# Liam-Eagen/BulletproofsPP

Measured on AMD Instinct MI355X. Metric: msm_scalar_point_pairs_per_sec, higher is better.
Workload: dtype u256 modular integer (Fq: 10x26-bit lazy limbs, Fr: 8x32-bit limbs); 1 GPU; pedersen_msm_2^20_secp256k1; pairs_per_gpu=1048576, window_bits=auto, algorithm=signed-digit Pippenger, affine in / XYZZ buckets

## Files before the change

bulletproofspp_amd/capi.py:

```python
from __future__ import annotations

import ctypes as C
import os
from typing import Optional, Sequence, Tuple

import numpy as np

_HERE = os.path.dirname(os.path.abspath(__file__))
NUM_STAGES = 6
STAGE_NAMES = ["digits", "sort", "acc_points", "acc_records", "reduce", "finish"]

SYMBOLS = [
    "bppp_ctx_create", "bppp_ctx_destroy", "bppp_ctx_set_stream", "bppp_last_error", "bppp_version",
    "bppp_msm", "bppp_msm_device", "bppp_msm_batch_device", "bppp_sum_points", "bppp_rational_reduce",
    "bppp_fold_points", "bppp_fold_points_device", "bppp_rational_reduce_eis", "bppp_fold_points_eis_device",
    "bppp_norm_round_sums_device", "bppp_lin_round_sums_device",
    "bppp_norm_round_openings_device", "bppp_lin_round_openings_device",
    "bppp_fold_scalars_device", "bppp_tensor_device", "bppp_batch_inverse_device",
    "bppp_nl_create", "bppp_nl_destroy", "bppp_nl_lengths", "bppp_nl_round_commit", "bppp_nl_round_collapse",
    "bppp_nl_get_witness", "bppp_nl_download", "bppp_nl_verify", "bppp_nl_verify_batch_device", "bppp_nl_prove", "bppp_nl_verify_challenges",
    "bppp_nlb_create", "bppp_nlb_destroy", "bppp_nlb_lengths", "bppp_nlb_round_commit", "bppp_nlb_round_collapse", "bppp_nlb_get_witness",
    "bppp_ip_create", "bppp_ip_destroy", "bppp_ip_lengths", "bppp_ip_round_commit", "bppp_ip_round_collapse", "bppp_ip_get_witness", "bppp_ip_verify", "bppp_ip_verify_batch_device",
    "bppp_lift_x_device", "bppp_device_alloc", "bppp_device_free", "bppp_upload", "bppp_download", "bppp_host_alloc", "bppp_host_free",
    "bppp_profile_enable", "bppp_profile_read",
# ... 214 lines not shown
    lib = C.CDLL(p)
    vp, sz, i = C.c_void_p, C.c_size_t, C.c_int
    lib.bppp_test_fe_op.argtypes = [vp, i, i, vp, vp, sz, vp]
    lib.bppp_test_point_op.argtypes = [vp, i, vp, vp, sz, vp]
    lib.bppp_test_point_quad.argtypes = [vp, i, vp, vp, sz, vp, vp]
    lib.bppp_test_fq_pair.argtypes = [vp, i, vp, vp, vp, vp, sz, vp]
    lib.bppp_test_point_chain.argtypes = [vp, i, vp, vp, sz, vp, vp]
    lib.bppp_test_mulmod_rate.argtypes = [vp, i, C.POINTER(C.c_double)]
    lib.bppp_test_last_mixed_msm_terms.argtypes = [vp, C.POINTER(C.c_uint64)]
    lib.bppp_test_last_sort_ranges.argtypes = [vp, C.POINTER(C.c_int)]
    lib.bppp_test_last_scatter_one_read.argtypes = [vp, C.POINTER(C.c_int)]
    lib.bppp_test_last_acc_sized.argtypes = [vp, C.POINTER(C.c_int)]
    lib.bppp_test_last_acc_fq29.argtypes = [vp, C.POINTER(C.c_int)]
    lib.bppp_test_fq29_op.argtypes = [vp, i, vp, vp, sz, vp, vp]
    lib.bppp_test_madd29_chain.argtypes = [vp, vp, vp, sz, sz, vp, vp]
    lib.bppp_test_last_windows.argtypes = [vp, C.POINTER(C.c_int)]
    lib.bppp_test_rp_last_verify_counts.argtypes = [vp, C.POINTER(C.c_uint64), C.POINTER(C.c_uint64)]
    lib.bppp_test_rp_last_block_counts.argtypes = [vp] + [C.POINTER(C.c_uint64)] * 4
    lib.bppp_test_rp_set_each_chunk.argtypes = [vp, sz]
    lib.bppp_test_rp_set_tally_short_max.argtypes = [vp, sz]
    lib.bppp_test_rp_set_tally_piece.argtypes = [vp, sz]
    lib.bppp_test_rp_set_tally_chunk.argtypes = [vp, sz]
    lib.bppp_test_rp_set_flat_chunk.argtypes = [vp, sz]
    lib.bppp_test_rp_excess_mul.argtypes = [vp, sz, vp, vp, vp]
    lib.bppp_test_rp_excess_mul2.argtypes = [vp, sz, vp, vp, vp, vp, vp]
    lib.bppp_test_rp_witness_device.argtypes = [vp, sz, vp, vp, vp, vp, vp, vp, vp, vp, vp]
    lib.bppp_test_points_from_seed_chunked.argtypes = [vp, C.c_char_p, sz, C.c_uint64, sz, sz, vp, C.POINTER(C.c_uint64)]
    lib.bppp_test_seed_lift_digests.argtypes = [vp, C.c_char_p, sz, vp, vp, vp]
    lib.bppp_test_rp_decode_device.argtypes = [vp, sz, C.c_char_p, C.c_char_p, vp, vp, vp, vp, vp, vp]
    lib.bppp_test_comb_create.argtypes = [vp, vp, sz, i, C.POINTER(vp)]
# ... 411 lines not shown
```

bulletproofspp_amd/csrc/capi.hip:

```cpp
#include <stdlib.h>
#include <string.h>
#include "ctx.hpp"
#include "hostmath.hpp"
#include "hosteis.hpp"

namespace bppp {
int msm_run(bppp_ctx *, const void *, const void *, size_t, size_t, int, int, uint64_t *);
int fold_points_run(bppp_ctx *, const uint64_t *, int, const uint64_t *, int, const void *, size_t, void *);
int norm_round_sums_run(bppp_ctx *, const void *, size_t, const uint64_t *, uint64_t *, uint64_t *);
int lin_round_sums_run(bppp_ctx *, const void *, const void *, size_t, uint64_t *, uint64_t *);
int round_openings_run(bppp_ctx *, const void *, size_t, int, const uint64_t *, const uint64_t *, void *, void *);
int fold_scalars_run(bppp_ctx *, const uint64_t *, const uint64_t *, const void *, size_t, void *);
int tensor_run(bppp_ctx *, const uint64_t *, size_t, const uint64_t *, const uint64_t *, size_t, void *);
int lift_x_run(bppp_ctx *, const void *, size_t, void *);
int batch_inverse_run(bppp_ctx *, const void *, size_t, int, void *);
int fold_points_eis_run(bppp_ctx *, const uint64_t *, const int *, const uint64_t *, const int *, const void *, size_t, void *);

void ctx_retain(bppp_ctx *ctx) { ctx->refs.fetch_add(1); }
void ctx_release(bppp_ctx *ctx) {
  if (ctx->refs.fetch_sub(1) != 1) return;
  hipSetDevice(ctx->device);
  hipStreamSynchronize(ctx->stream);
  if (ctx->aux_stream) hipStreamSynchronize(ctx->aux_stream);
  if (ctx->ws) hipFree(ctx->ws);
// ... 20 lines not shown
  lacc = env_int("BPPP_LACC", 0);
  window_batched = env_int("BPPP_WINDOW_BATCHED", 0);
  comb_wpe = env_int("BPPP_COMB_WPE", 0);
  comb_rows_waves = env_int("BPPP_COMB_ROWS_WAVES", 0);
  if (const char *e = getenv("BPPP_COMB_ROWS_MIN_MB")) comb_rows_min_bytes = (size_t)strtoull(e, nullptr, 10) << 20;
  small_c = env_int("BPPP_MSM_SMALL_C", 0);
  small_len = env_int("BPPP_MSM_SMALL_LEN", 0);
  small_max = env_int("BPPP_MSM_SMALL_MAX", 0);
  hist_ch = env_int("BPPP_HIST_CH", 0);
  no_small = env_flag("BPPP_MSM_NO_SMALL");
  no_balance = env_flag("BPPP_MSM_NO_BALANCE");
  sort_ranges = env_int("BPPP_SORT_RANGES", sort_ranges);
  scatter_one_read = env_switch("BPPP_SCATTER_ONE_READ", scatter_one_read);
  acc_sized = env_switch("BPPP_ACC_SIZED", acc_sized);
  acc_fq29 = env_switch("BPPP_ACC_FQ29", acc_fq29);
}
namespace bppp {
int ctx_aux(bppp_ctx *ctx) {
  if (ctx->aux_stream) return BPPP_OK;
  BPPP_HIP(ctx, hipStreamCreateWithFlags(&ctx->aux_stream, hipStreamNonBlocking));
  BPPP_HIP(ctx, hipEventCreateWithFlags(&ctx->aux_fork, hipEventDisableTiming));
  BPPP_HIP(ctx, hipEventCreateWithFlags(&ctx->aux_join, hipEventDisableTiming));
  return BPPP_OK;
}
void ctx_drain(bppp_ctx *ctx) {
  if (ctx_closed(ctx)) return;
  hipStreamSynchronize(ctx->stream);
  if (ctx->aux_stream) hipStreamSynchronize(ctx->aux_stream);
  (void)hipGetLastError();
}
// ... 289 lines not shown
```

bulletproofspp_amd/csrc/ctx.hpp:

```cpp
#pragma once
#include <hip/hip_runtime.h>
#include <stdint.h>
#include <atomic>
#include <string>
#include <vector>
#include "../../include/bppp.h"
#include "msm_plan.hpp"

struct CombLast {
  int route = -1;
  int heavy_first = 0;
  uint32_t parts = 0, tparts = 0, wsplit = 0;
  uint32_t chunks = 0, clen = 0, join_lanes = 0;
};

struct bppp_ctx {
  MsmTune tune;
  std::atomic<int> refs{1};
  std::atomic<bool> closed{false};
  int device = 0;
  hipStream_t stream = nullptr;
  hipStream_t own_stream = nullptr;
  hipStream_t aux_stream = nullptr;
  hipEvent_t aux_fork = nullptr, aux_join = nullptr;
// ... 6 lines not shown
  void *pre_acc_arg = nullptr;
  void *pinned = nullptr;
  size_t pinned_bytes = 0;
  bool profile = false;
  double stage_ms[BPPP_NUM_STAGES] = {0, 0, 0, 0, 0, 0};
  uint64_t calls = 0;
  hipEvent_t ev[BPPP_NUM_STAGES + 1] = {};
  bool ev_ready = false;
  void *mix = nullptr;
  size_t mix_bytes = 0;
  uint64_t last_mixed_terms = 0;
  int last_sort_ranges = -1;
  int last_scatter_one_read = -1;
  int last_acc_sized = -1;
  int last_acc_fq29 = -1;
  int last_windows = -1;
  CombLast last_comb;
  size_t sort_lds_set = 0;
};

namespace bppp {

inline int fail(bppp_ctx *ctx, int code, const std::string &msg) {
  if (ctx) ctx->err = msg;
  return code;
}
#define BPPP_HIP(ctx, call)                                                                    \
  do {                                                                                         \
    hipError_t _e = (call);                                                                    \
    if (_e != hipSuccess)                                                                      \
// ... 16 lines not shown
```

bulletproofspp_amd/csrc/ec29.hip.h:

```cpp
#pragma once
#include "ec.hip.h"
#include "fq29.hip.h"

namespace bppp {

struct aff29 { fq29 x, y; };
struct xyzz29 { fq29 X, Y, ZZ, ZZZ; };

BPPP_DI bool aff29_is_inf(const aff29 &p) { return fq29_all_zero(p.x) && fq29_all_zero(p.y); }
BPPP_DI bool xyzz29_is_inf(const xyzz29 &p) { return fq29_all_zero(p.ZZ); }
BPPP_DI xyzz29 xyzz29_inf() { xyzz29 r; r.X = fq29_zero(); r.Y = fq29_zero(); r.ZZ = fq29_zero(); r.ZZZ = fq29_zero(); return r; }
BPPP_DI xyzz29 xyzz29_from_aff(const aff29 &p) {
  xyzz29 r; r.X = p.x; r.Y = p.y;
  r.ZZ = fq29_zero(); r.ZZ.n[0] = aff29_is_inf(p) ? 0u : 1u; r.ZZZ = r.ZZ;
  return r;
}
BPPP_DI aff29 aff29_cneg(const aff29 &p, bool neg) {
  aff29 r; r.x = p.x;
  const fq29 ny = fq29_neg<1>(p.y);
  const bool inf = aff29_is_inf(p);
#pragma unroll
  for (int i = 0; i < 9; i++) r.y.n[i] = (neg && !inf) ? ny.n[i] : p.y.n[i];
  return r;
}
// ... 18 lines not shown
  if (fq29_weak_is_zero(Pd)) {
    if (fq29_weak_is_zero(R)) acc = xyzz29_dbl_aff(q); else acc = xyzz29_inf();
    return;
  }
  const fq29 PP = fq29_sqr(Pd), PPP = fq29_mul(Pd, PP), Q = fq29_mul(acc.X, PP);
  const fq29 X3 = fq29_sub<3>(fq29_sqr(R), fq29_add(PPP, fq29_mul_int(Q, 2)));
  const fq29 Y3 = fq29_sub<1>(fq29_mul(R, fq29_sub<5>(Q, X3)), fq29_mul(acc.Y, PPP));
  acc.ZZ = fq29_mul(acc.ZZ, PP); acc.ZZZ = fq29_mul(acc.ZZZ, PPP);
  acc.X = X3; acc.Y = Y3;
}

BPPP_DI xyzz xyzz29_to_xyzz(const xyzz29 &a) {
  xyzz r; r.X = fq29_to_fq26(a.X); r.Y = fq29_to_fq26(a.Y); r.ZZ = fq29_to_fq26(a.ZZ); r.ZZZ = fq29_to_fq26(a.ZZZ);
  return r;
}

}
```

bulletproofspp_amd/csrc/fq26.hip.h:

```cpp
#pragma once
#include "fe.hip.h"
#include "modinv.hip.h"

namespace bppp {

struct fq { uint32_t n[10]; };

static constexpr uint32_t FQ_M26 = 0x3FFFFFFu, FQ_M22 = 0x3FFFFFu;
static constexpr uint32_t FQ_R0 = 0x3D10u, FQ_R1 = 0x400u;

BPPP_DI uint32_t fq_plimb(int i) { return i == 0 ? 0x3FFFC2Fu : i == 1 ? 0x3FFFFBFu : i == 9 ? FQ_M22 : FQ_M26; }

BPPP_DI fq fq_zero() { fq r; for (int i = 0; i < 10; i++) r.n[i] = 0; return r; }
BPPP_DI fq fq_one() { fq r = fq_zero(); r.n[0] = 1; return r; }
BPPP_DI bool fq_all_zero(const fq &a) {
  uint32_t o = 0;
#pragma unroll
  for (int i = 0; i < 10; i++) o |= a.n[i];
  return o == 0;
}

BPPP_DI uint64_t fq_madc(uint32_t x, uint32_t y, uint64_t acc) { uint64_t r = (uint64_t)x * y + acc; asm("" : "+v"(r)); return r; }
BPPP_DI uint32_t fq_sreg(uint32_t v) { asm("" : "+s"(v)); return v; }
BPPP_DI void fq_mul_tail(fq &r, uint64_t c, uint32_t t9, uint64_t u9, uint32_t u8) {
  c += (uint64_t)t9 + u9 * FQ_R0 + (uint64_t)u8 * FQ_R1;
  r.n[9] = (uint32_t)c & FQ_M22;
  const uint64_t top = (c >> 22) + ((u9 * FQ_R1) << 4);
  c = (uint64_t)r.n[0] + top * 0x3D1u; r.n[0] = (uint32_t)c & FQ_M26; c >>= 26;
  c += (uint64_t)r.n[1] + (top << 6); r.n[1] = (uint32_t)c & FQ_M26; c >>= 26;
  c += r.n[2]; r.n[2] = (uint32_t)c & FQ_M26; c >>= 26;
  r.n[3] += (uint32_t)c;
}
BPPP_DI fq fq_mul(const fq &a, const fq &b) {
  const uint32_t R0 = fq_sreg(FQ_R0), R1 = fq_sreg(FQ_R1);
  uint64_t d = 0;
#pragma unroll
  for (int i = 0; i <= 9; i++) d = fq_madc(a.n[i], b.n[9 - i], d);
  const uint32_t t9 = (uint32_t)d & FQ_M26; d >>= 26;
// ... 47 lines not shown
    if (k) c = fq_madc(u[k - 1], R1, c);
    r.n[k] = (uint32_t)c & FQ_M26; c >>= 26;
  }
  fq_mul_tail(r, c, t9, u9, u[8]);
  return r;
}

template <bool SQ> BPPP_DI constexpr int fq_col_n(int k) {
  return SQ ? ((k + 1) / 2 - (k > 9 ? k - 9 : 0)) + ((k & 1) == 0 ? 1 : 0) : (k < 9 ? k : 9) - (k > 9 ? k - 9 : 0) + 1;
}
template <bool SQ> BPPP_DI uint64_t fq_col_step(const fq &a, const fq &b, int k, int j, uint64_t acc) {
  const int i = (k > 9 ? k - 9 : 0) + j;
  if (SQ) return 2 * i < k ? fq_madc(b.n[i], a.n[k - i], acc) : fq_madc(a.n[k / 2], a.n[k / 2], acc);
  return fq_madc(a.n[i], b.n[k - i], acc);
}
BPPP_DI void fq_fence() { __builtin_amdgcn_sched_barrier(0); }
template <bool SQ1, bool SQ2> BPPP_DI void fq_pair(const fq a, const fq b_, const fq c, const fq d_, fq &r1, fq &r2) {
  const uint32_t R0 = fq_sreg(FQ_R0), R1 = fq_sreg(FQ_R1);
  fq b = b_, d = d_;
#pragma unroll
  for (int i = 0; i < 10; i++) { if (SQ1) b.n[i] = a.n[i] << 1; if (SQ2) d.n[i] = c.n[i] << 1; }
  uint64_t h1 = 0, h2 = 0;
  uint32_t t9a = 0, t9b = 0, u1[9], u2[9];
#pragma unroll
  for (int k = 9; k <= 18; k++) {
#pragma unroll
    for (int j = 0; j < 10; j++) {
      if (j < fq_col_n<SQ1>(k)) { h1 = fq_col_step<SQ1>(a, b, k, j, h1); fq_fence(); }
      if (j < fq_col_n<SQ2>(k)) { h2 = fq_col_step<SQ2>(c, d, k, j, h2); fq_fence(); }
    }
    if (k == 9) { t9a = (uint32_t)h1 & FQ_M26; t9b = (uint32_t)h2 & FQ_M26; }
// ... 227 lines not shown
```

bulletproofspp_amd/csrc/fq29.hip.h:

```cpp
#pragma once
#include "fq26.hip.h"

namespace bppp {

struct fq29 { uint32_t n[9]; };

static constexpr uint32_t FQ29_M29 = 0x1FFFFFFFu, FQ29_M24 = 0xFFFFFFu;
static constexpr uint32_t FQ29_R0 = 0x7A20u, FQ29_R1 = 0x100u;

BPPP_DI uint32_t fq29_plimb(int i) { return i == 0 ? 0x1FFFFC2Fu : i == 1 ? 0x1FFFFFF7u : i == 8 ? FQ29_M24 : FQ29_M29; }

BPPP_DI fq29 fq29_zero() { fq29 r; for (int i = 0; i < 9; i++) r.n[i] = 0; return r; }
BPPP_DI bool fq29_all_zero(const fq29 &a) {
  uint32_t o = 0;
#pragma unroll
  for (int i = 0; i < 9; i++) o |= a.n[i];
  return o == 0;
}

BPPP_DI void fq29_mul_tail(fq29 &r, uint64_t c, uint32_t t8, uint64_t u8, uint32_t u7) {
  c += (uint64_t)t8 + u8 * FQ29_R0 + (uint64_t)u7 * FQ29_R1;
  r.n[8] = (uint32_t)c & FQ29_M24;
  const uint64_t top = (c >> 24) + ((u8 * FQ29_R1) << 5);
  c = (uint64_t)r.n[0] + top * 0x3D1u; r.n[0] = (uint32_t)c & FQ29_M29; c >>= 29;
// ... 48 lines not shown
    u[k - 9] = (uint32_t)d & FQ29_M29; d >>= 29;
  }
  const uint64_t u8 = d;
  fq29 r;
  uint64_t c = 0;
#pragma unroll
  for (int k = 0; k < 8; k++) {
    FQ29_SQCHAIN(c, k)
    c = fq_madc(u[k], R0, c);
    if (k) c = fq_madc(u[k - 1], R1, c);
    r.n[k] = (uint32_t)c & FQ29_M29; c >>= 29;
  }
  fq29_mul_tail(r, c, t8, u8, u[7]);
  return r;
}

BPPP_DI fq29 fq29_add(const fq29 &a, const fq29 &b) {
  fq29 r;
#pragma unroll
  for (int i = 0; i < 9; i++) r.n[i] = a.n[i] + b.n[i];
  return r;
}
template <int K> BPPP_DI fq29 fq29_neg(const fq29 &a) {
  fq29 r;
#pragma unroll
  for (int i = 0; i < 9; i++) r.n[i] = (uint32_t)(K + 1) * fq29_plimb(i) - a.n[i];
  return r;
}
template <int K> BPPP_DI fq29 fq29_sub(const fq29 &a, const fq29 &b) {
  fq29 r;
// ... 44 lines not shown
  const fq29 t = fq29_weak_pass(a);
  fq r;
  r.n[0] = t.n[0] & FQ_M26;
  r.n[1] = ((t.n[0] >> 26) | (t.n[1] << 3)) & FQ_M26;
  r.n[2] = ((t.n[1] >> 23) | (t.n[2] << 6)) & FQ_M26;
  r.n[3] = ((t.n[2] >> 20) | (t.n[3] << 9)) & FQ_M26;
  r.n[4] = ((t.n[3] >> 17) | (t.n[4] << 12)) & FQ_M26;
  r.n[5] = ((t.n[4] >> 14) | (t.n[5] << 15)) & FQ_M26;
  r.n[6] = ((t.n[5] >> 11) | (t.n[6] << 18)) & FQ_M26;
  r.n[7] = ((t.n[6] >> 8) | (t.n[7] << 21)) & FQ_M26;
  r.n[8] = ((t.n[7] >> 5) | (t.n[8] << 24)) & FQ_M26;
  r.n[9] = t.n[8] >> 2;
  return r;
}

BPPP_DI void fq29_store9(uint32_t *p, const fq29 &a) {
#pragma unroll
  for (int i = 0; i < 9; i++) p[i] = a.n[i];
}
BPPP_DI fq29 fq29_load9(const uint32_t *p) {
  fq29 r;
#pragma unroll
  for (int i = 0; i < 9; i++) r.n[i] = p[i];
  return r;
}

}
```

bulletproofspp_amd/csrc/msm.hip:

```cpp
#include <algorithm>
#include <vector>
#include "ctx.hpp"
#include "ec.hip.h"
#include "ec29.hip.h"
#include "ec_quad.hip.h"
#include "hostcurve.hpp"
#include "hostmath.hpp"
#include "recode.hip.h"

namespace bppp {

static_assert(MSM_XYZZ_WORDS == XYZZ_WORDS, "msm_plan.hpp sizes the workspace by the stored point of ec.hip.h");
static_assert(sizeof(MsmPair) == sizeof(uint2) && sizeof(MsmQuad) == sizeof(uint4) && alignof(MsmQuad) == alignof(uint4), "the workspace's pairs and quadruples are the kernels' uint2 / uint4");

__global__ void __launch_bounds__(256) k_digits(const uint32_t *__restrict__ scalars, uint64_t total, uint32_t n, uint32_t stride, int c,
                                                int W, int acnt, int top, RecodeK K, uint16_t *__restrict__ dig,
                                                unsigned long long *__restrict__ negmask, uint32_t *__restrict__ zero, uint32_t nzero,
                                                uint32_t *__restrict__ zero2, uint32_t nzero2) {
  uint64_t i = (uint64_t)blockIdx.x * blockDim.x + threadIdx.x;
  for (uint64_t j = i; j < nzero; j += (uint64_t)gridDim.x * blockDim.x) zero[j] = 0u;
  for (uint64_t j = i; j < nzero2; j += (uint64_t)gridDim.x * blockDim.x) zero2[j] = 0u;
  bool valid = i < total;
  bool neg = false;
  if (valid) {
// ... 530 lines not shown
  for (int d = 1; d < 64; d <<= 1) {
    xyzz o = xyzz_shfl_down(suf, d);
    if ((int)lane + d < 64) xyzz_add(suf, o);
  }
  xyzz v = (lane >= 1) ? suf : xyzz_inf();
  for (int k = 64 * Lw; k > 1; k >>= 1) v = xyzz_dbl(v);
  xyzz_add(v, A);
  for (int d = 32; d >= 1; d >>= 1) {
    xyzz o = xyzz_shfl_down(v, d);
    if ((int)lane + d < 64) xyzz_add(v, o);
  }
  if (lane == 0) xyzz_store(winsum + (size_t)nbw * XYZZ_WORDS, v);
}


BPPP_DI xyzz marg_serial_sum(const uint32_t *b, int S, size_t stride) {
  xyzz acc = xyzz_load(b);
  if (S < 2) return acc;
  xyzz B = xyzz_load(b + stride);
  for (int k = 2; k < S; k++) {
    const xyzz Bn = xyzz_load(b + (size_t)k * stride);
    xyzz_add_chain(acc, B);
    B = Bn;
  }
  xyzz_add_chain(acc, B);
  return acc;
}

__global__ void __launch_bounds__(64) k_reduce_marg(const uint32_t *__restrict__ buckets, int M, MargGeom Gm, uint32_t *__restrict__ R, uint32_t *__restrict__ C) {
  const uint32_t nbw = blockIdx.y, lane = threadIdx.x;
  const uint32_t *wb = buckets + (size_t)nbw * M * XYZZ_WORDS;
  xyzz acc = xyzz_inf();
  if (blockIdx.x < Gm.row_tiles) {
    const uint32_t r = blockIdx.x * 64 + lane, hi = r / (uint32_t)Gm.PR, part = r % (uint32_t)Gm.PR;
    const bool act = hi < (uint32_t)Gm.HI;
    if (act) {
      const uint32_t *b = wb + ((size_t)hi * Gm.LO + (size_t)part * Gm.SR) * XYZZ_WORDS;
      acc = marg_serial_sum(b, Gm.SR, XYZZ_WORDS);
    }
    for (int d = Gm.PR >> 1; d >= 1; d >>= 1) {
      xyzz o = xyzz_shfl_down(acc, d);
      if ((int)part + d < Gm.PR) xyzz_add_chain(acc, o);
    }
    if (act && part == 0) xyzz_store(R + ((size_t)nbw * Gm.HI + hi) * XYZZ_WORDS, acc);
  } else {
    const uint32_t q = (blockIdx.x - Gm.row_tiles) * 64 + lane, lo = q / (uint32_t)Gm.PC, part = q % (uint32_t)Gm.PC;
    const bool act = lo < (uint32_t)Gm.LO;
    if (act) {
      const uint32_t *b = wb + ((size_t)part * Gm.SC * Gm.LO + lo) * XYZZ_WORDS;
      acc = marg_serial_sum(b, Gm.SC, (size_t)Gm.LO * XYZZ_WORDS);
    }
    for (int d = Gm.PC >> 1; d >= 1; d >>= 1) {
      xyzz o = xyzz_shfl_down(acc, d);
      if ((int)part + d < Gm.PC) xyzz_add_chain(acc, o);
    }
    if (act && part == 0) xyzz_store(C + ((size_t)nbw * Gm.LO + lo) * XYZZ_WORDS, acc);
  }
}

__global__ void __launch_bounds__(64) k_reduce_tail_quad(const uint32_t *__restrict__ R, const uint32_t *__restrict__ C, MargGeom Gm, uint32_t *__restrict__ part,
                                                         uint32_t *__restrict__ cnt, uint32_t *__restrict__ winsum2) {
  __shared__ uint32_t last;
  const uint32_t nbw = blockIdx.y, lane = threadIdx.x, qd = lane >> 2;
  const bool isC = blockIdx.x >= (uint32_t)Gm.TR;
  const uint32_t blk = isC ? blockIdx.x - Gm.TR : blockIdx.x, nb = isC ? Gm.TC : Gm.TR, i = blk * 16 + qd;
  xyzz suf = xyzz_inf();
  if (isC) suf = xyzz_load(C + ((size_t)nbw * Gm.LO + i) * XYZZ_WORDS);
  else if (i + 1 < (uint32_t)Gm.HI) suf = xyzz_load(R + ((size_t)nbw * Gm.HI + i + 1) * XYZZ_WORDS);
  for (int d = 1; d < 16; d <<= 1) {
    xyzz o = xyzz_shfl_down(suf, 4 * d);
    xyzz_add_quad<true>(suf, xyzz_or_inf(qd + d < 16, o));
  }
// ... 287 lines not shown
                                                         ws.heavy_count, ws.chunk_sums);
  } else {
    k_acc_points<<<dim3((unsigned)((p.G + 255) / 256)), dim3(256), 0, st>>>(ws.sorted, ws.start, (uint32_t)p.FB, (const uint32_t *)d_points, (uint32_t)p.n,
                                                                            (uint32_t)(p.Wc * p.M), shared_points, p.L, p.G, ws.buckets, ws.rec_pt);
    prof_mark(ctx, 3);
    k_merge<<<dim3((unsigned)((p.FB + 255) / 256)), dim3(256), 0, st>>>(ws.start, ws.count, p.FB, p.L, ws.rec_pt, ws.buckets, heavy_items, ws.heavy_slot, heavy_buckets,
                                                                        ws.heavy_count);
    k_merge_heavy<false><<<dim3(2048), dim3(64), 0, st>>>(ws.start, ws.count, p.L, ws.rec_pt, nullptr, ws.buckets, heavy_items, ws.heavy_slot, heavy_buckets,
                                                          ws.heavy_count, ws.chunk_sums);
  }
  return BPPP_OK;
}

static void msm_reduce(bppp_ctx *ctx, const MsmPlan &p, const MsmWorkspace &ws) {
  hipStream_t st = ctx->stream;
  if (p.RG) {
    k_reduce_groups<<<dim3((unsigned)((p.NS * p.RG + 63) / 64)), dim3(64), 0, st>>>(ws.buckets, p.M, p.RG, (uint32_t)p.NS, ws.winsum);
  } else if (p.marg) {
    uint32_t *Rm = ws.red, *Cm = ws.red + (size_t)p.NS * p.mg.HI * XYZZ_WORDS;
    k_reduce_marg<<<dim3(p.mg.row_tiles + p.mg.col_tiles, (unsigned)p.NS), dim3(64), 0, st>>>(ws.buckets, p.M, p.mg, Rm, Cm);
    k_reduce_tail_quad<<<dim3((unsigned)(p.mg.TR + p.mg.TC), (unsigned)p.NS), dim3(64), 0, st>>>(Rm, Cm, p.mg, ws.tail_part, ws.tail_cnt, ws.winsum);
  } else {
    k_reduce1<<<dim3((unsigned)p.NS, p.WPW), dim3(64), 0, st>>>(ws.buckets, p.M, p.Lw, p.WPW, ws.red);
    k_reduce2<<<dim3((unsigned)p.NS), dim3(64), 0, st>>>(ws.red, p.Lw, p.WPW, ws.winsum);
  }
}

static int msm_finish(bppp_ctx *ctx, const MsmPlan &p, const MsmWorkspace &ws, uint64_t *out_xy, uint32_t *d_out_dev) {
  using namespace bppp_host;
  hipStream_t st = ctx->stream;
  const size_t batch = p.batch;
  const int a = p.marg ? p.mg.a : 0;
  if (d_out_dev) {
    k_window_combine<<<dim3((unsigned)((batch + 63) / 64)), dim3(64), 0, st>>>(ws.winsum, p.Wc, p.c, a, (uint32_t)batch, d_out_dev);
    BPPP_HIP(ctx, hipGetLastError());
// ... 70 lines not shown
```

bulletproofspp_amd/csrc/msm_plan.hpp:

```cpp
#pragma once
#include <stddef.h>
#include <stdint.h>
#include <string.h>
#include <algorithm>

struct MsmTune {
  double gcost = 0;
  int cmin = 0;
  int lw = 0;
  int rg = 0;
  int marg_s = 0;
  int lacc = 0;
  int window_batched = 0;
  int comb_wpe = 0;
  int small_c = 0;
  int small_len = 0;
  int small_max = 0;
  int hist_ch = 0;
  int num_cus = 0;
  int sort_ranges = 4;
  int scatter_one_read = 1;
  int acc_sized = -1;
  int acc_fq29 = 1;
  bool no_small = false;
  bool no_balance = false;
  size_t comb_rows_min_bytes = (size_t)4 << 30;
  int comb_rows_waves = 0;
  void from_env();
};

namespace bppp {

struct Carver {
  char *base; size_t off = 0, cap;
  Carver(void *b, size_t c) : base((char *)b), cap(c) {}
  template <typename T> T *take(size_t count) {
    size_t bytes = (count * sizeof(T) + 255) & ~(size_t)255;
    T *p = (T *)(base ? base + off : nullptr);
// ... 246 lines not shown
```

bulletproofspp_amd/csrc/testhooks.hip:

```cpp
#include "../../include/bppp_test.h"
#include <vector>
#include "ctx.hpp"
#include "ec.hip.h"
#include "ec29.hip.h"
#include "ec_quad.hip.h"
#include "modinv.hip.h"
#include "fr26.hip.h"
#include "rp_internal.hpp"
#include "rpwitness.hip.h"
#include "rpdecode.hip.h"
#include "rpexcess.hip.h"
#include "rpexpart.hip.h"
#include "seedpoints.hip.h"
#include "comb.hip.h"
#include "rpp_transcript.hpp"

namespace bppp {
template <int MOD> BPPP_DI fe apply_op(int op, const fe &a, const fe &b) {
  switch (op) {
    case BPPP_FE_ADD: return fe_add<MOD>(a, b);
    case BPPP_FE_SUB: return fe_sub<MOD>(a, b);
    case BPPP_FE_MUL: return fe_mul<MOD>(a, b);
    case BPPP_FE_SQR: return fe_sqr<MOD>(a);
    case BPPP_FE_INV: return fe_inv<MOD>(a);
// ... 145 lines not shown
  const fq t = fq29_to_fq26(r);
  fq29_store9(raw + (size_t)i * 19, r);
  fq_store10(raw + (size_t)i * 19 + 9, t);
  fe_store(out + (size_t)i * 8, fq_to_fe(t));
}
__global__ void __launch_bounds__(64) k_test_madd29_chain(const uint32_t *pts, const uint32_t *flags, uint32_t k, uint32_t n, uint32_t *out, uint32_t *raw) {
  const uint32_t i = blockIdx.x * 64 + threadIdx.x;
  if (i >= n) return;
  const uint32_t *p = pts + (size_t)i * k * 16, *f = flags + (size_t)i * k;
  xyzz29 acc = xyzz29_from_aff(aff29_cneg(aff29_load(p), f[0] != 0));
  for (uint32_t j = 1; j < k; j++) xyzz29_madd(acc, aff29_cneg(aff29_load(p + (size_t)j * 16), f[j] != 0));
  const xyzz s = xyzz29_to_xyzz(acc);
  xyzz_store(raw + (size_t)i * XYZZ_WORDS, s);
  aff_store(out + (size_t)i * 16, xyzz_to_aff(s));
}
}

using namespace bppp;

static int run2(bppp_ctx *ctx, const uint64_t *a, const uint64_t *b, size_t n, size_t words, uint64_t *out, void **da, void **db, void **dout) {
  size_t bytes = n * words * 8;
  BPPP_HIP(ctx, hipMalloc(da, bytes)); BPPP_HIP(ctx, hipMalloc(db, bytes)); BPPP_HIP(ctx, hipMalloc(dout, bytes));
  BPPP_HIP(ctx, hipMemcpyAsync(*da, a, bytes, hipMemcpyHostToDevice, ctx->stream));
  BPPP_HIP(ctx, hipMemcpyAsync(*db, b, bytes, hipMemcpyHostToDevice, ctx->stream));
  (void)out;
  return BPPP_OK;
}

extern "C" int bppp_test_fe_op(bppp_ctx *ctx, int op, int modulus, const uint64_t *a, const uint64_t *b, size_t n, uint64_t *out) {
  if (!ctx || !a || !b || !out) return BPPP_ERR_ARG;
// ... 164 lines not shown
}
extern "C" int bppp_test_madd29_chain(bppp_ctx *ctx, const uint64_t *points, const uint32_t *flags, size_t k, size_t n, uint64_t *out, uint32_t *raw) {
  if (!ctx || !points || !flags || !out || !raw || !k || k >= (1u << 16) || n >= (1u << 16)) return BPPP_ERR_ARG;
  if (n == 0) return BPPP_OK;
  hipSetDevice(ctx->device);
  uint32_t *d = nullptr;
  if (hipMalloc(&d, (n * k * 17 + n * (16 + XYZZ_WORDS)) * 4) != hipSuccess) return bppp::fail(ctx, BPPP_ERR_HIP, "test_madd29_chain: hipMalloc");
  uint32_t *d_f = d + n * k * 16, *d_out = d_f + n * k, *d_raw = d_out + n * 16;
  hipStream_t st = ctx->stream;
  bool ok = hipMemcpyAsync(d, points, n * k * 64, hipMemcpyHostToDevice, st) == hipSuccess && hipMemcpyAsync(d_f, flags, n * k * 4, hipMemcpyHostToDevice, st) == hipSuccess;
  if (ok) k_test_madd29_chain<<<dim3((unsigned)((n + 63) / 64)), dim3(64), 0, st>>>(d, d_f, (uint32_t)k, (uint32_t)n, d_out, d_raw);
  ok = ok && hipMemcpyAsync(out, d_out, n * 64, hipMemcpyDeviceToHost, st) == hipSuccess && hipMemcpyAsync(raw, d_raw, n * XYZZ_WORDS * 4, hipMemcpyDeviceToHost, st) == hipSuccess;
  if (hipStreamSynchronize(st) != hipSuccess) ok = false;
  hipFree(d);
  return ok ? BPPP_OK : bppp::fail(ctx, BPPP_ERR_HIP, "test_madd29_chain: kernel or copy failed");
}

extern "C" int bppp_test_last_windows(bppp_ctx *ctx, int *windows) {
  if (!ctx || !windows) return BPPP_ERR_ARG;
  *windows = ctx->last_windows;
  return BPPP_OK;
}

extern "C" int bppp_test_rp_last_verify_counts(bppp_rp *rp, uint64_t *combined_msms, uint64_t *each_passes) {
  if (!rp || !combined_msms || !each_passes) return BPPP_ERR_ARG;
  *combined_msms = rp->n_combined;
  *each_passes = rp->n_each;
  return BPPP_OK;
}

// ... 312 lines not shown
```

Measured before the change: 838.2 million pairs/s.

## Run marginal bucket reduction in 9x29-bit limb arithmetic with paired multiplies

Adds a 29-bit-limb variant of the marginal bucket-reduction kernel. Buckets are repacked from the 10x26-bit format into 9x29-bit limbs, summed with a new XYZZ add chain built on interleaved paired modular multiplies, and converted back on store. Fewer limbs mean fewer partial products per multiply, and pairing two independent multiplies gives the scheduler more instruction-level parallelism. In exchange it adds repacking cost per bucket load and output, plus more code to keep correct. The path is on by default through a tuning switch.

Measured after the change: 839.1 million pairs/s (median of 3 runs). Within noise of the previous version (+0.1%).

```diff
diff --git a/bulletproofspp_amd/capi.py b/bulletproofspp_amd/capi.py
--- a/bulletproofspp_amd/capi.py
+++ b/bulletproofspp_amd/capi.py
@@ -252,6 +252,10 @@
     lib.bppp_test_last_acc_fq29.argtypes = [vp, C.POINTER(C.c_int)]
     lib.bppp_test_fq29_op.argtypes = [vp, i, vp, vp, sz, vp, vp]
     lib.bppp_test_madd29_chain.argtypes = [vp, vp, vp, sz, sz, vp, vp]
+    lib.bppp_test_last_reduce_fq29.argtypes = [vp, C.POINTER(C.c_int)]
+    lib.bppp_test_fq29_pair.argtypes = [vp, i, vp, sz, vp]
+    lib.bppp_test_fq29_repack.argtypes = [vp, vp, sz, vp]
+    lib.bppp_test_add29_chain.argtypes = [vp, i, vp, sz, vp, vp]
     lib.bppp_test_last_windows.argtypes = [vp, C.POINTER(C.c_int)]
     lib.bppp_test_rp_last_verify_counts.argtypes = [vp, C.POINTER(C.c_uint64), C.POINTER(C.c_uint64)]
     lib.bppp_test_rp_last_block_counts.argtypes = [vp] + [C.POINTER(C.c_uint64)] * 4
diff --git a/bulletproofspp_amd/csrc/capi.hip b/bulletproofspp_amd/csrc/capi.hip
--- a/bulletproofspp_amd/csrc/capi.hip
+++ b/bulletproofspp_amd/csrc/capi.hip
@@ -58,6 +58,7 @@
   scatter_one_read = env_switch("BPPP_SCATTER_ONE_READ", scatter_one_read);
   acc_sized = env_switch("BPPP_ACC_SIZED", acc_sized);
   acc_fq29 = env_switch("BPPP_ACC_FQ29", acc_fq29);
+  reduce_fq29 = env_switch("BPPP_REDUCE_FQ29", reduce_fq29);
 }
 namespace bppp {
 int ctx_aux(bppp_ctx *ctx) {
diff --git a/bulletproofspp_amd/csrc/ctx.hpp b/bulletproofspp_amd/csrc/ctx.hpp
--- a/bulletproofspp_amd/csrc/ctx.hpp
+++ b/bulletproofspp_amd/csrc/ctx.hpp
@@ -44,6 +44,7 @@
   int last_scatter_one_read = -1;
   int last_acc_sized = -1;
   int last_acc_fq29 = -1;
+  int last_reduce_fq29 = -1;
   int last_windows = -1;
   CombLast last_comb;
   size_t sort_lds_set = 0;
diff --git a/bulletproofspp_amd/csrc/ec29.hip.h b/bulletproofspp_amd/csrc/ec29.hip.h
--- a/bulletproofspp_amd/csrc/ec29.hip.h
+++ b/bulletproofspp_amd/csrc/ec29.hip.h
@@ -56,5 +56,50 @@
   xyzz r; r.X = fq29_to_fq26(a.X); r.Y = fq29_to_fq26(a.Y); r.ZZ = fq29_to_fq26(a.ZZ); r.ZZZ = fq29_to_fq26(a.ZZZ);
   return r;
 }
+BPPP_DI xyzz29 xyzz29_from_xyzz(const xyzz &a) {
+  xyzz29 r; r.X = fq29_from_fq26_limbs(a.X); r.Y = fq29_from_fq26_limbs(a.Y); r.ZZ = fq29_from_fq26_limbs(a.ZZ); r.ZZZ = fq29_from_fq26_limbs(a.ZZZ);
+  return r;
+}
+
+BPPP_DI xyzz29 xyzz29_dbl_via26(const xyzz29 &p) {
+  const xyzz d = xyzz_dbl_chain(xyzz29_to_xyzz(p));
+  xyzz29 r; r.X = fq29_from_fq26(d.X); r.Y = fq29_from_fq26(d.Y); r.ZZ = fq29_from_fq26(d.ZZ); r.ZZZ = fq29_from_fq26(d.ZZZ);
+  return r;
+}
+BPPP_DI void xyzz29_add_chain(xyzz29 &acc, const xyzz29 &q) {
+  if (xyzz29_is_inf(q)) return;
+  if (xyzz29_is_inf(acc)) { acc = q; return; }
+  fq29 U1, U2, S1, S2;
+  fq29_mul2(acc.X, q.ZZ, q.X, acc.ZZ, U1, U2);
+  fq29_mul2(acc.Y, q.ZZZ, q.Y, acc.ZZZ, S1, S2);
+  const fq29 Pd = fq29_weak_pass(fq29_sub<1>(U2, U1));
+  const fq29 R = fq29_weak_pass(fq29_sub<1>(S2, S1));
+  if (fq29_weak_is_zero(Pd)) {
+    if (fq29_weak_is_zero(R)) acc = xyzz29_dbl_via26(acc); else acc = xyzz29_inf();
+    return;
+  }
+  fq29 PP, RR, Z12, Z123, PPP, Q, Ya, Yb;
+  fq29_sqr2(Pd, R, PP, RR);
+  fq29_mul2(acc.ZZ, q.ZZ, acc.ZZZ, q.ZZZ, Z12, Z123);
+  fq29_mul2(Pd, PP, U1, PP, PPP, Q);
+  xyzz29 r;
+  r.X = fq29_sub<3>(RR, fq29_add(PPP, fq29_mul_int(Q, 2)));
+  fq29_mul2(Z12, PP, Z123, PPP, r.ZZ, r.ZZZ);
+  fq29_mul2(R, fq29_sub<5>(Q, r.X), S1, PPP, Ya, Yb);
+  r.Y = fq29_sub<1>(Ya, Yb);
+  acc = r;
+}
+
+BPPP_DI fq29 fq29_shfl_down(const fq29 &a, int d) {
+  fq29 r;
+#pragma unroll
+  for (int i = 0; i < 9; i++) r.n[i] = (uint32_t)__shfl_down((int)a.n[i], d, 64);
+  return r;
+}
+BPPP_DI xyzz29 xyzz29_shfl_down(const xyzz29 &p, int d) {
+  xyzz29 r; r.X = fq29_shfl_down(p.X, d); r.Y = fq29_shfl_down(p.Y, d);
+  r.ZZ = fq29_shfl_down(p.ZZ, d); r.ZZZ = fq29_shfl_down(p.ZZZ, d);
+  return r;
+}
 
 }
diff --git a/bulletproofspp_amd/csrc/fq26.hip.h b/bulletproofspp_amd/csrc/fq26.hip.h
--- a/bulletproofspp_amd/csrc/fq26.hip.h
+++ b/bulletproofspp_amd/csrc/fq26.hip.h
@@ -20,8 +20,17 @@
   return o == 0;
 }
 
+#ifdef BPPP_FQ_HOST_CHECK
+BPPP_DI uint64_t fq_madc(uint32_t x, uint32_t y, uint64_t acc) {
+  const unsigned __int128 r = (unsigned __int128)((uint64_t)x * y) + acc;
+  if (r >> 64) BPPP_FQ_HOST_CHECK("fq_madc");
+  return (uint64_t)r;
+}
+BPPP_DI uint32_t fq_sreg(uint32_t v) { return v; }
+#else
 BPPP_DI uint64_t fq_madc(uint32_t x, uint32_t y, uint64_t acc) { uint64_t r = (uint64_t)x * y + acc; asm("" : "+v"(r)); return r; }
 BPPP_DI uint32_t fq_sreg(uint32_t v) { asm("" : "+s"(v)); return v; }
+#endif
 BPPP_DI void fq_mul_tail(fq &r, uint64_t c, uint32_t t9, uint64_t u9, uint32_t u8) {
   c += (uint64_t)t9 + u9 * FQ_R0 + (uint64_t)u8 * FQ_R1;
   r.n[9] = (uint32_t)c & FQ_M22;
@@ -99,7 +108,11 @@
   if (SQ) return 2 * i < k ? fq_madc(b.n[i], a.n[k - i], acc) : fq_madc(a.n[k / 2], a.n[k / 2], acc);
   return fq_madc(a.n[i], b.n[k - i], acc);
 }
+#ifdef BPPP_FQ_HOST_CHECK
+BPPP_DI void fq_fence() {}
+#else
 BPPP_DI void fq_fence() { __builtin_amdgcn_sched_barrier(0); }
+#endif
 template <bool SQ1, bool SQ2> BPPP_DI void fq_pair(const fq a, const fq b_, const fq c, const fq d_, fq &r1, fq &r2) {
   const uint32_t R0 = fq_sreg(FQ_R0), R1 = fq_sreg(FQ_R1);
   fq b = b_, d = d_;
diff --git a/bulletproofspp_amd/csrc/fq29.hip.h b/bulletproofspp_amd/csrc/fq29.hip.h
--- a/bulletproofspp_amd/csrc/fq29.hip.h
+++ b/bulletproofspp_amd/csrc/fq29.hip.h
@@ -86,6 +86,59 @@
   fq29_mul_tail(r, c, t8, u8, u[7]);
   return r;
 }
+
+template <bool SQ> BPPP_DI constexpr int fq29_col_n(int k) {
+  return SQ ? ((k + 1) / 2 - (k > 8 ? k - 8 : 0)) + ((k & 1) == 0 ? 1 : 0) : (k < 8 ? k : 8) - (k > 8 ? k - 8 : 0) + 1;
+}
+template <bool SQ> BPPP_DI uint64_t fq29_col_step(const fq29 &a, const fq29 &b, int k, int j, uint64_t acc) {
+  const int i = (k > 8 ? k - 8 : 0) + j;
+  if (SQ) return 2 * i < k ? fq_madc(b.n[i], a.n[k - i], acc) : fq_madc(a.n[k / 2], a.n[k / 2], acc);
+  return fq_madc(a.n[i], b.n[k - i], acc);
+}
+BPPP_DI void fq29_opaque(fq29 &a) {
+#ifndef BPPP_FQ_HOST_CHECK
+#pragma unroll
+  for (int i = 0; i < 9; i++) asm volatile("" : "+v"(a.n[i]));
+#endif
+}
+template <bool SQ1, bool SQ2> BPPP_DI void fq29_pair(const fq29 a, const fq29 b_, const fq29 c, const fq29 d_, fq29 &r1, fq29 &r2) {
+  const uint32_t R0 = fq_sreg(FQ29_R0), R1 = fq_sreg(FQ29_R1);
+  fq29 b = b_, d = d_;
+#pragma unroll
+  for (int i = 0; i < 9; i++) { if (SQ1) b.n[i] = a.n[i] << 1; if (SQ2) d.n[i] = c.n[i] << 1; }
+  uint64_t h1 = 0, h2 = 0;
+  uint32_t t8a = 0, t8b = 0, u1[8], u2[8];
+#pragma unroll
+  for (int k = 8; k <= 16; k++) {
+#pragma unroll
+    for (int j = 0; j < 9; j++) {
+      if (j < fq29_col_n<SQ1>(k)) { h1 = fq29_col_step<SQ1>(a, b, k, j, h1); fq_fence(); }
+      if (j < fq29_col_n<SQ2>(k)) { h2 = fq29_col_step<SQ2>(c, d, k, j, h2); fq_fence(); }
+    }
+    if (k == 8) { t8a = (uint32_t)h1 & FQ29_M29; t8b = (uint32_t)h2 & FQ29_M29; }
+    else { u1[k - 9] = (uint32_t)h1 & FQ29_M29; u2[k - 9] = (uint32_t)h2 & FQ29_M29; }
+    h1 >>= 29; h2 >>= 29;
+  }
+  uint64_t l1 = 0, l2 = 0;
+#pragma unroll
+  for (int k = 0; k < 8; k++) {
+#pragma unroll
+    for (int j = 0; j < 8; j++) {
+      if (j < fq29_col_n<SQ1>(k)) { l1 = fq29_col_step<SQ1>(a, b, k, j, l1); fq_fence(); }
+      if (j < fq29_col_n<SQ2>(k)) { l2 = fq29_col_step<SQ2>(c, d, k, j, l2); fq_fence(); }
+    }
+    l1 = fq_madc(u1[k], R0, l1); fq_fence(); l2 = fq_madc(u2[k], R0, l2); fq_fence();
+    if (k) { l1 = fq_madc(u1[k - 1], R1, l1); fq_fence(); l2 = fq_madc(u2[k - 1], R1, l2); fq_fence(); }
+    r1.n[k] = (uint32_t)l1 & FQ29_M29; l1 >>= 29;
+    r2.n[k] = (uint32_t)l2 & FQ29_M29; l2 >>= 29;
+  }
+  fq29_mul_tail(r1, l1, t8a, h1, u1[7]);
+  fq29_mul_tail(r2, l2, t8b, h2, u2[7]);
+  fq29_opaque(r1); fq29_opaque(r2);
+}
+BPPP_DI void fq29_mul2(const fq29 &a, const fq29 &b, const fq29 &c, const fq29 &d, fq29 &r1, fq29 &r2) { fq29_pair<false, false>(a, b, c, d, r1, r2); }
+BPPP_DI void fq29_mul_sqr(const fq29 &a, const fq29 &b, const fq29 &c, fq29 &r1, fq29 &r2) { fq29_pair<false, true>(a, b, c, c, r1, r2); }
+BPPP_DI void fq29_sqr2(const fq29 &a, const fq29 &c, fq29 &r1, fq29 &r2) { fq29_pair<true, true>(a, a, c, c, r1, r2); }
 
 BPPP_DI fq29 fq29_add(const fq29 &a, const fq29 &b) {
   fq29 r;
@@ -160,6 +213,22 @@
   return r;
 }
 
+BPPP_DI fq29 fq29_from_fq26_limbs(const fq &a) {
+  const uint32_t x = a.n[9] >> 22;
+  fq29 r;
+  uint64_t c = (uint64_t)a.n[0] + (uint64_t)x * 0x3D1u + ((uint64_t)(a.n[1] + (x << 6)) << 26);
+  r.n[0] = (uint32_t)c & FQ29_M29; c >>= 29; c += (uint64_t)a.n[2] << 23;
+  r.n[1] = (uint32_t)c & FQ29_M29; c >>= 29; c += (uint64_t)a.n[3] << 20;
+  r.n[2] = (uint32_t)c & FQ29_M29; c >>= 29; c += (uint64_t)a.n[4] << 17;
+  r.n[3] = (uint32_t)c & FQ29_M29; c >>= 29; c += (uint64_t)a.n[5] << 14;
+  r.n[4] = (uint32_t)c & FQ29_M29; c >>= 29; c += (uint64_t)a.n[6] << 11;
+  r.n[5] = (uint32_t)c & FQ29_M29; c >>= 29; c += (uint64_t)a.n[7] << 8;
+  r.n[6] = (uint32_t)c & FQ29_M29; c >>= 29; c += (uint64_t)a.n[8] << 5;
+  r.n[7] = (uint32_t)c & FQ29_M29; c >>= 29; c += (uint64_t)(a.n[9] & FQ_M22) << 2;
+  r.n[8] = (uint32_t)c;
+  return r;
+}
+
 BPPP_DI void fq29_store9(uint32_t *p, const fq29 &a) {
 #pragma unroll
   for (int i = 0; i < 9; i++) p[i] = a.n[i];
diff --git a/bulletproofspp_amd/csrc/msm.hip b/bulletproofspp_amd/csrc/msm.hip
--- a/bulletproofspp_amd/csrc/msm.hip
+++ b/bulletproofspp_amd/csrc/msm.hip
@@ -568,48 +568,70 @@
 }
 
 
-BPPP_DI xyzz marg_serial_sum(const uint32_t *b, int S, size_t stride) {
-  xyzz acc = xyzz_load(b);
+struct MargFq26 {
+  typedef xyzz pt;
+  static BPPP_DI xyzz inf() { return xyzz_inf(); }
+  static BPPP_DI xyzz unpack(const xyzz &s) { return s; }
+  static BPPP_DI void add(xyzz &acc, const xyzz &q) { xyzz_add_chain(acc, q); }
+  static BPPP_DI xyzz shfl_down(const xyzz &p, int d) { return xyzz_shfl_down(p, d); }
+  static BPPP_DI xyzz stored(const xyzz &acc) { return acc; }
+};
+struct MargFq29 {
+  typedef xyzz29 pt;
+  static BPPP_DI xyzz29 inf() { return xyzz29_inf(); }
+  static BPPP_DI xyzz29 unpack(const xyzz &s) { return xyzz29_from_xyzz(s); }
+  static BPPP_DI void add(xyzz29 &acc, const xyzz29 &q) { xyzz29_add_chain(acc, q); }
+  static BPPP_DI xyzz29 shfl_down(const xyzz29 &p, int d) { return xyzz29_shfl_down(p, d); }
+  static BPPP_DI xyzz stored(const xyzz29 &acc) { return xyzz29_to_xyzz(acc); }
+};
+template <class A> BPPP_DI typename A::pt marg_serial_sum(const uint32_t *b, int S, size_t stride) {
+  typename A::pt acc = A::unpack(xyzz_load(b));
   if (S < 2) return acc;
   xyzz B = xyzz_load(b + stride);
   for (int k = 2; k < S; k++) {
     const xyzz Bn = xyzz_load(b + (size_t)k * stride);
-    xyzz_add_chain(acc, B);
+    A::add(acc, A::unpack(B));
     B = Bn;
   }
-  xyzz_add_chain(acc, B);
+  A::add(acc, A::unpack(B));
   return acc;
 }
 
-__global__ void __launch_bounds__(64) k_reduce_marg(const uint32_t *__restrict__ buckets, int M, MargGeom Gm, uint32_t *__restrict__ R, uint32_t *__restrict__ C) {
+template <class A> BPPP_DI void reduce_marg(const uint32_t *__restrict__ buckets, int M, const MargGeom &Gm, uint32_t *__restrict__ R, uint32_t *__restrict__ C) {
   const uint32_t nbw = blockIdx.y, lane = threadIdx.x;
   const uint32_t *wb = buckets + (size_t)nbw * M * XYZZ_WORDS;
-  xyzz acc = xyzz_inf();
+  typename A::pt acc = A::inf();
   if (blockIdx.x < Gm.row_tiles) {
     const uint32_t r = blockIdx.x * 64 + lane, hi = r / (uint32_t)Gm.PR, part = r % (uint32_t)Gm.PR;
     const bool act = hi < (uint32_t)Gm.HI;
     if (act) {
       const uint32_t *b = wb + ((size_t)hi * Gm.LO + (size_t)part * Gm.SR) * XYZZ_WORDS;
-      acc = marg_serial_sum(b, Gm.SR, XYZZ_WORDS);
+      acc = marg_serial_sum<A>(b, Gm.SR, XYZZ_WORDS);
     }
     for (int d = Gm.PR >> 1; d >= 1; d >>= 1) {
-      xyzz o = xyzz_shfl_down(acc, d);
-      if ((int)part + d < Gm.PR) xyzz_add_chain(acc, o);
-    }
-    if (act && part == 0) xyzz_store(R + ((size_t)nbw * Gm.HI + hi) * XYZZ_WORDS, acc);
+      typename A::pt o = A::shfl_down(acc, d);
+      if ((int)part + d < Gm.PR) A::add(acc, o);
+    }
+    if (act && part == 0) xyzz_store(R + ((size_t)nbw * Gm.HI + hi) * XYZZ_WORDS, A::stored(acc));
   } else {
     const uint32_t q = (blockIdx.x - Gm.row_tiles) * 64 + lane, lo = q / (uint32_t)Gm.PC, part = q % (uint32_t)Gm.PC;
     const bool act = lo < (uint32_t)Gm.LO;
     if (act) {
       const uint32_t *b = wb + ((size_t)part * Gm.SC * Gm.LO + lo) * XYZZ_WORDS;
-      acc = marg_serial_sum(b, Gm.SC, (size_t)Gm.LO * XYZZ_WORDS);
+      acc = marg_serial_sum<A>(b, Gm.SC, (size_t)Gm.LO * XYZZ_WORDS);
     }
     for (int d = Gm.PC >> 1; d >= 1; d >>= 1) {
-      xyzz o = xyzz_shfl_down(acc, d);
-      if ((int)part + d < Gm.PC) xyzz_add_chain(acc, o);
-    }
-    if (act && part == 0) xyzz_store(C + ((size_t)nbw * Gm.LO + lo) * XYZZ_WORDS, acc);
-  }
+      typename A::pt o = A::shfl_down(acc, d);
+      if ((int)part + d < Gm.PC) A::add(acc, o);
+    }
+    if (act && part == 0) xyzz_store(C + ((size_t)nbw * Gm.LO + lo) * XYZZ_WORDS, A::stored(acc));
+  }
+}
+__global__ void __launch_bounds__(64) k_reduce_marg(const uint32_t *__restrict__ buckets, int M, MargGeom Gm, uint32_t *__restrict__ R, uint32_t *__restrict__ C) {
+  reduce_marg<MargFq26>(buckets, M, Gm, R, C);
+}
+__global__ void __launch_bounds__(64) k_reduce_marg29(const uint32_t *__restrict__ buckets, int M, MargGeom Gm, uint32_t *__restrict__ R, uint32_t *__restrict__ C) {
+  reduce_marg<MargFq29>(buckets, M, Gm, R, C);
 }
 
 __global__ void __launch_bounds__(64) k_reduce_tail_quad(const uint32_t *__restrict__ R, const uint32_t *__restrict__ C, MargGeom Gm, uint32_t *__restrict__ part,
@@ -927,11 +949,14 @@
 
 static void msm_reduce(bppp_ctx *ctx, const MsmPlan &p, const MsmWorkspace &ws) {
   hipStream_t st = ctx->stream;
+  ctx->last_reduce_fq29 = 0;
   if (p.RG) {
     k_reduce_groups<<<dim3((unsigned)((p.NS * p.RG + 63) / 64)), dim3(64), 0, st>>>(ws.buckets, p.M, p.RG, (uint32_t)p.NS, ws.winsum);
   } else if (p.marg) {
     uint32_t *Rm = ws.red, *Cm = ws.red + (size_t)p.NS * p.mg.HI * XYZZ_WORDS;
-    k_reduce_marg<<<dim3(p.mg.row_tiles + p.mg.col_tiles, (unsigned)p.NS), dim3(64), 0, st>>>(ws.buckets, p.M, p.mg, Rm, Cm);
+    const bool fq29 = ctx->tune.reduce_fq29 != 0;
+    ctx->last_reduce_fq29 = fq29 ? 1 : 0;
+    (fq29 ? k_reduce_marg29 : k_reduce_marg)<<<dim3(p.mg.row_tiles + p.mg.col_tiles, (unsigned)p.NS), dim3(64), 0, st>>>(ws.buckets, p.M, p.mg, Rm, Cm);
     k_reduce_tail_quad<<<dim3((unsigned)(p.mg.TR + p.mg.TC), (unsigned)p.NS), dim3(64), 0, st>>>(Rm, Cm, p.mg, ws.tail_part, ws.tail_cnt, ws.winsum);
   } else {
     k_reduce1<<<dim3((unsigned)p.NS, p.WPW), dim3(64), 0, st>>>(ws.buckets, p.M, p.Lw, p.WPW, ws.red);
diff --git a/bulletproofspp_amd/csrc/msm_plan.hpp b/bulletproofspp_amd/csrc/msm_plan.hpp
--- a/bulletproofspp_amd/csrc/msm_plan.hpp
+++ b/bulletproofspp_amd/csrc/msm_plan.hpp
@@ -22,6 +22,7 @@
   int scatter_one_read = 1;
   int acc_sized = -1;
   int acc_fq29 = 1;
+  int reduce_fq29 = 1;
   bool no_small = false;
   bool no_balance = false;
   size_t comb_rows_min_bytes = (size_t)4 << 30;
diff --git a/bulletproofspp_amd/csrc/testhooks.hip b/bulletproofspp_amd/csrc/testhooks.hip
--- a/bulletproofspp_amd/csrc/testhooks.hip
+++ b/bulletproofspp_amd/csrc/testhooks.hip
@@ -183,6 +183,44 @@
   xyzz_store(raw + (size_t)i * XYZZ_WORDS, s);
   aff_store(out + (size_t)i * 16, xyzz_to_aff(s));
 }
+__global__ void __launch_bounds__(64) k_test_fq29_pair(int kind, const uint32_t *a, const uint32_t *b, const uint32_t *c, const uint32_t *d, uint32_t n, uint32_t *raw) {
+  const uint32_t i = blockIdx.x * 64 + threadIdx.x;
+  if (i >= n) return;
+  const fq29 A = fq29_load9(a + (size_t)i * 9), B = fq29_load9(b + (size_t)i * 9), Cc = fq29_load9(c + (size_t)i * 9), D = fq29_load9(d + (size_t)i * 9);
+  fq29 r1, r2, s1, s2;
+  if (kind == 0) { fq29_mul2(A, B, Cc, D, r1, r2); s1 = fq29_mul(A, B); s2 = fq29_mul(Cc, D); }
+  else if (kind == 1) { fq29_mul_sqr(A, B, Cc, r1, r2); s1 = fq29_mul(A, B); s2 = fq29_sqr(Cc); }
+  else { fq29_sqr2(A, Cc, r1, r2); s1 = fq29_sqr(A); s2 = fq29_sqr(Cc); }
+  uint32_t *o = raw + (size_t)i * 36;
+  fq29_store9(o, r1); fq29_store9(o + 9, r2); fq29_store9(o + 18, s1); fq29_store9(o + 27, s2);
+}
+__global__ void __launch_bounds__(64) k_test_fq29_repack(const uint32_t *a, uint32_t n, uint32_t *raw) {
+  const uint32_t i = blockIdx.x * 64 + threadIdx.x;
+  if (i >= n) return;
+  const fq29 r = fq29_from_fq26_limbs(fq_load10(a + (size_t)i * 10));
+  fq29_store9(raw + (size_t)i * 19, r);
+  fq_store10(raw + (size_t)i * 19 + 9, fq29_to_fq26(r));
+}
+__global__ void __launch_bounds__(64) k_test_add29_chain(int op, const uint32_t *p, const uint32_t *q, uint32_t n, uint32_t *out, uint32_t *raw) {
+  const uint32_t i = blockIdx.x * 64 + threadIdx.x;
+  if (i >= n) return;
+  const aff P = aff_load(p + (size_t)i * 16), Q = aff_load(q + (size_t)i * 16);
+  xyzz A = xyzz_from_aff(P), B = xyzz_from_aff(Q);
+  if (op & 1) { A = xyzz_dbl_aff(P); xyzz_madd(A, P); }
+  if (op & 2) { B = xyzz_dbl_aff(Q); xyzz_madd(B, Q); }
+  xyzz29 r = xyzz29_from_xyzz(A), b29 = xyzz29_from_xyzz(B);
+  if (op & 4) {
+    r.X = fq29_sub<3>(r.X, fq29_zero()); r.Y = fq29_sub<1>(r.Y, fq29_zero());
+    b29.X = fq29_sub<3>(b29.X, fq29_zero()); b29.Y = fq29_sub<1>(b29.Y, fq29_zero());
+  }
+  xyzz29_add_chain(r, b29);
+  xyzz s = A;
+  xyzz_add_chain(s, B);
+  const xyzz st = xyzz29_to_xyzz(r);
+  xyzz_store(raw + (size_t)i * XYZZ_WORDS, st);
+  aff_store(out + (size_t)i * 32, xyzz_to_aff(st));
+  aff_store(out + (size_t)i * 32 + 16, xyzz_to_aff(s));
+}
 }
 
 using namespace bppp;
@@ -377,6 +415,50 @@
   if (hipStreamSynchronize(st) != hipSuccess) ok = false;
   hipFree(d);
   return ok ? BPPP_OK : bppp::fail(ctx, BPPP_ERR_HIP, "test_madd29_chain: kernel or copy failed");
+}
+
+extern "C" int bppp_test_last_reduce_fq29(bppp_ctx *ctx, int *fq29) {
+  if (!ctx || !fq29) return BPPP_ERR_ARG;
+  *fq29 = ctx->last_reduce_fq29;
+  return BPPP_OK;
+}
+template <class F> static int run_words(bppp_ctx *ctx, const char *what, const uint32_t *in, size_t in_words, uint32_t *outp, size_t out_words, F launch) {
+  hipSetDevice(ctx->device);
+  uint32_t *d = nullptr;
+  if (hipMalloc(&d, (in_words + out_words) * 4) != hipSuccess) return bppp::fail(ctx, BPPP_ERR_HIP, what);
+  hipStream_t st = ctx->stream;
+  bool ok = hipMemcpyAsync(d, in, in_words * 4, hipMemcpyHostToDevice, st) == hipSuccess;
+  if (ok) launch(d, d + in_words, st);
+  ok = ok && hipMemcpyAsync(outp, d + in_words, out_words * 4, hipMemcpyDeviceToHost, st) == hipSuccess;
+  if (hipStreamSynchronize(st) != hipSuccess) ok = false;
+  hipFree(d);
+  return ok ? BPPP_OK : bppp::fail(ctx, BPPP_ERR_HIP, what);
+}
+extern "C" int bppp_test_fq29_pair(bppp_ctx *ctx, int kind, const uint32_t *abcd, size_t n, uint32_t *raw) {
+  if (!ctx || !abcd || !raw || kind < 0 || kind > 2 || n >= (1u << 20)) return BPPP_ERR_ARG;
+  if (n == 0) return BPPP_OK;
+  return run_words(ctx, "test_fq29_pair", abcd, n * 36, raw, n * 36, [&](uint32_t *in, uint32_t *o, hipStream_t st) {
+    k_test_fq29_pair<<<dim3((unsigned)((n + 63) / 64)), dim3(64), 0, st>>>(kind, in, in + n * 9, in + n * 18, in + n * 27, (uint32_t)n, o);
+  });
+}
+extern "C" int bppp_test_fq29_repack(bppp_ctx *ctx, const uint32_t *a, size_t n, uint32_t *raw) {
+  if (!ctx || !a || !raw || n >= (1u << 20)) return BPPP_ERR_ARG;
+  if (n == 0) return BPPP_OK;
+  return run_words(ctx, "test_fq29_repack", a, n * 10, raw, n * 19, [&](uint32_t *in, uint32_t *o, hipStream_t st) {
+    k_test_fq29_repack<<<dim3((unsigned)((n + 63) / 64)), dim3(64), 0, st>>>(in, (uint32_t)n, o);
+  });
+}
+extern "C" int bppp_test_add29_chain(bppp_ctx *ctx, int op, const uint64_t *pq, size_t n, uint64_t *out, uint32_t *raw) {
+  if (!ctx || !pq || !out || !raw || op < 0 || op > 7 || n >= (1u << 20)) return BPPP_ERR_ARG;
+  if (n == 0) return BPPP_OK;
+  std::vector<uint32_t> back(n * (32 + XYZZ_WORDS));
+  int rc = run_words(ctx, "test_add29_chain", (const uint32_t *)pq, n * 32, back.data(), back.size(), [&](uint32_t *in, uint32_t *o, hipStream_t st) {
+    k_test_add29_chain<<<dim3((unsigned)((n + 63) / 64)), dim3(64), 0, st>>>(op, in, in + n * 16, (uint32_t)n, o, o + n * 32);
+  });
+  if (rc) return rc;
+  memcpy(out, back.data(), n * 32 * 4);
+  memcpy(raw, back.data() + n * 32, n * XYZZ_WORDS * 4);
+  return BPPP_OK;
 }
 
 extern "C" int bppp_test_last_windows(bppp_ctx *ctx, int *windows) {
```
